# migoox/genome-downsampler

Measured on AMD Instinct MI355X. Metric: Mreads/s selected at target coverage M=100, higher is better.
Workload: dtype u32

## Files before the change

### genome-downsampler_amd/__init__.py

```python
import contextlib
import ctypes as C
import fractions
import heapq
import math
import numbers
import operator
import os

import numpy as np

_HERE = os.path.dirname(os.path.abspath(__file__))
LIB_DIR = os.path.join(_HERE, "lib")
HIP_LIB_PATH = os.environ.get("QMCP_HIP_LIB") or os.path.join(LIB_DIR, "libqmcp_hip.so")
HOST_LIB_PATH = os.environ.get("QMCP_HOST_LIB") or os.path.join(LIB_DIR, "libqmcp_host.so")

ABI_SYMBOLS = (
    "qmcp_hip_abi_version", "qmcp_hip_last_error", "qmcp_hip_device_count", "qmcp_hip_create",
    "qmcp_hip_destroy", "qmcp_hip_solve_host", "qmcp_hip_solve_device", "qmcp_hip_coverage_host",
    "qmcp_hip_filtered_coverage_host", "qmcp_hip_complete_pairs_device",
    "qmcp_hip_complete_pairs_host", "qmcp_hip_amplicon_filter_host", "qmcp_hip_set_profiling",
    "qmcp_hip_kernel_times", "qmcp_hip_filter_solve_host", "qmcp_hip_solve_device_begin",
    "qmcp_hip_solve_end", "qmcp_hip_demand_host", "qmcp_hip_solve_host64", "qmcp_hip_multi_create",
    "qmcp_hip_multi_destroy", "qmcp_hip_multi_solve_host", "qmcp_hip_kept_indices_host",
    "qmcp_hip_default_options", "qmcp_hip_set_options", "qmcp_hip_get_options",
# ... 52 lines not shown
NO_TIER = 0xFFFFFFFF
TIERS_MAX = 16
STRATUM_TALLY_TILE = 1024


QMCP_OK, QMCP_EINVAL, QMCP_EREAD, QMCP_ERANGE, QMCP_ENODEVICE, QMCP_EHIP, QMCP_ENOMEM = 0, -1, -2, -3, -4, -5, -6


class QmcpError(RuntimeError):
    def __init__(self, code, message):
        super().__init__(f"qmcp_hip error {code}: {message}")
        self.code = code


class HostBreakdown(C.Structure):
    _fields_ = [("ms_total", C.c_float), ("ms_narrow_h2d", C.c_float), ("ms_solve", C.c_float),
                ("ms_d2h", C.c_float), ("host_threads", C.c_uint32), ("chunks", C.c_uint32),
                ("columns_sent", C.c_uint32)]


class Stats(C.Structure):
    _fields_ = [
        ("n_reads", C.c_uint64), ("n_kept", C.c_uint64), ("total_length", C.c_uint64),
        ("n_contigs", C.c_uint32), ("path", C.c_uint32), ("min_span", C.c_uint32),
        ("max_span", C.c_uint32), ("sort_passes", C.c_uint32), ("sweep_stretches", C.c_uint32),
        ("ms_total", C.c_float), ("ms_prepare", C.c_float), ("ms_scan", C.c_float),
        ("ms_sort", C.c_float), ("ms_sweep", C.c_float), ("ms_mark", C.c_float),
        ("ms_h2d", C.c_float), ("ms_d2h", C.c_float), ("columns_sent", C.c_uint32),
        ("spec_boundaries", C.c_uint32), ("spec_mismatches", C.c_uint32),
        ("spec_retry_mismatches", C.c_uint32), ("sweep_blocks_changed", C.c_uint32), ("sweep_blocks", C.c_uint32),
        ("arena_grown_mid_solve", C.c_uint32), ("near_uniform_exceptions", C.c_uint32),
        ("near_uniform_selected", C.c_uint32), ("near_uniform_rounds", C.c_uint32),
        ("near_uniform_giveup", C.c_uint32), ("pm_grid", C.c_int32), ("pm_heaviest_wave_slots", C.c_uint32),
    ]

    def as_dict(self):
        return {name: getattr(self, name) for name, _ in self._fields_}


class QualityStats(C.Structure):
    _fields_ = [("quality_min", C.c_uint32), ("quality_max", C.c_uint32), ("key_bits", C.c_uint32),
                ("sort_passes", C.c_uint32), ("cells_contested", C.c_uint64), ("reads_swapped", C.c_uint64),
                ("ms_quality", C.c_float)]

    def as_dict(self):
        return {name: getattr(self, name) for name, _ in self._fields_}


class TargetStats(C.Structure):
    _fields_ = [("reads_on_target", C.c_uint64), ("reads_off_target", C.c_uint64), ("target_positions", C.c_uint64),
                ("regions_in", C.c_uint32), ("regions_merged", C.c_uint32), ("ms_targets", C.c_float)]

    def as_dict(self):
        return {name: getattr(self, name) for name, _ in self._fields_}


class ProfileStats(C.Structure):
    _fields_ = [("positions_in_regions", C.c_uint64), ("capped_positions", C.c_uint64), ("demand", C.c_uint64),
                ("regions_in", C.c_uint32), ("regions_used", C.c_uint32), ("ms_profile", C.c_float)]

    def as_dict(self):
        return {name: getattr(self, name) for name, _ in self._fields_}


class CeilingStats(C.Structure):
    _fields_ = [("reads_placed", C.c_uint64), ("reads_dropped", C.c_uint64), ("mates_dropped", C.c_uint64),
# ... 264 lines not shown


class AmpliconsStats(C.Structure):
    _fields_ = [("units", C.c_uint64), ("units_assigned", C.c_uint64), ("units_filtered", C.c_uint64),
                ("units_no_amplicon", C.c_uint64), ("units_in_several", C.c_uint64), ("reads_shortened", C.c_uint64),
                ("reads_clipped_away", C.c_uint64), ("bases_clipped", C.c_uint64), ("amplicons", C.c_uint64),
                ("amplicons_unused", C.c_uint64), ("ms_assign", C.c_float), ("ms_report", C.c_float)]

    def as_dict(self):
        return {name: getattr(self, name) for name, _ in self._fields_}


assert C.sizeof(AmpliconsStats) == 10 * 8 + 2 * 4


class DepthReport:

    def __init__(self, contig_rows, region_rows, hist_in, hist_kept, stats):
        self.contig_rows, self.region_rows = contig_rows, region_rows
        self.hist_in, self.hist_kept, self.stats = hist_in, hist_kept, stats

    @property
    def valid(self):
        return self.stats.deficit_positions == 0


class Options(C.Structure):
    _fields_ = [
        ("struct_size", C.c_uint32), ("pass_major", C.c_int32), ("sweep", C.c_int32), ("cut_points", C.c_int32),
        ("speculation", C.c_int32), ("speculation_run_in", C.c_uint32), ("near_uniform", C.c_int32),
        ("near_uniform_rounds", C.c_uint32), ("near_uniform_min_depth", C.c_float), ("near_uniform_debug", C.c_int32),
        ("force_sort_route", C.c_int32), ("keep_expand", C.c_int32), ("mixed_sweep_in_lds", C.c_int32),
        ("rank_min_reads", C.c_uint32), ("host_threads", C.c_uint32), ("copy_streams", C.c_uint32),
        ("host_both_columns", C.c_int32), ("pm_grid", C.c_int32),
    ]


class DownsampleRequest(C.Structure):
    _fields_ = (
        [("struct_size", C.c_uint64)]
        + [(name, C.c_char_p) for name in ("solver_name", "in_path", "out_path", "filtered_path", "bed", "tsv", "targets",
                                           "report", "track", "track_channel")]
        + [("ladder_levels", C.POINTER(C.c_uint32))]
        + [(name, C.c_char_p) for name in ("ladder_template", "stratify", "strata_report", "dedup_report")]
        + [(name, C.POINTER(C.c_uint32)) for name in ("region_offsets", "region_starts", "region_ends", "region_caps")]
        + [("n_refs", C.c_uint64), ("pair_stages", C.POINTER(C.c_uint32)), ("template_stages", C.POINTER(C.c_uint32)),
           ("fragment_report", C.c_char_p), ("ceiling_report", C.c_char_p), ("budget_report", C.c_char_p),
           ("budget_reads", C.c_uint64), ("budget_fraction", C.c_double), ("mean_depth_targets", C.c_char_p),
           ("mean_depth_report", C.c_char_p), ("budget_bases", C.c_uint64), ("mean_depth", C.c_double),
           ("thresholds_tag", C.c_char_p), ("thresholds_report", C.c_char_p),
           ("replicates_further", C.POINTER(C.c_uint32)),
           ("replicates_template", C.c_char_p), ("replicates_report", C.c_char_p)]
        + [(name, C.c_uint32) for name in ("max_coverage", "min_len", "min_mapq", "target_padding", "report_bins",
                                           "track_cap", "n_ladder_levels", "default_cap", "n_pair_stages",
                                           "n_template_stages", "n_replicates_further", "thresholds_lo",
                                           "thresholds_hi")]
        + [(name, C.c_int32) for name in ("amplicon_mode", "per_reference", "amplicons_by_reference", "keep_off_target",
                                          "dedup", "has_regions", "pair_aware", "template_aware", "split_spliced",
                                          "include_secondary", "fragment_depth", "ceiling", "has_budget_reads",
                                          "has_budget_bases", "has_mean_depth", "has_replicates", "has_thresholds",
                                          "start_cap_by_strand")]
        + [("start_cap", C.c_uint32), ("start_cap_report", C.c_char_p)]
        + [("primer_clip", C.c_int32), ("per_amplicon", C.c_int32), ("amplicon_report", C.c_char_p)]
        + [("mapq_tiers", C.POINTER(C.c_uint32)), ("n_mapq_tiers", C.c_uint32), ("tiers_report", C.c_char_p)]
        + [("proportional_report", C.c_char_p), ("proportion_num", C.c_uint32), ("proportion_den", C.c_uint32),
           ("proportion_floor", C.c_uint32), ("has_proportion", C.c_int32)])

# ... 2333 lines not shown
```

### genome-downsampler_amd/csrc/api/solve_head.inc.hip

```cpp
int queue_rm_head(qmcp_hip_ctx* c, hipStream_t s1, uint32_t filter, bool clear_mask);
int queue_pm_head(qmcp_hip_ctx* c, hipStream_t st, uint32_t filter, bool rerun);

bool pm_route_ok(const qmcp_hip_ctx* c, const uint64_t* roff, const Problem& pr, uint32_t shift, const qmcp::PmGridPlan& grid) {
    if (c->opt.pass_major < 0) return false;
    const uint32_t n = (uint32_t)pr.n;
    if ((uint64_t)qmcp::pm_slots(n, grid.n_ranges) >= (1ull << 31)) return false;
    if (c->opt.pass_major > 0) return true;
    double slots = 0.0;
    for (uint32_t k = 0; k < pr.n_contigs; ++k) {
        const uint64_t reads = roff[k + 1] - roff[k];
        if (reads == 0 || pr.poff[k + 1] == pr.poff[k]) continue;
        const double ranges = grid.aligned ? (double)((pr.poff[k + 1] - pr.poff[k] + ((1ull << shift) - 1)) >> shift)
                                           : (double)(((pr.poff[k + 1] - 1) >> shift) - (pr.poff[k] >> shift) + 1);
        const double passes = (double)reads / (double)qmcp::pm_pass() < 1.0 ? 1.0 : (double)reads / (double)qmcp::pm_pass();
        const double slice = (double)reads / (passes * ranges);
        slots += passes * ranges * std::ceil(slice / 64.0);
    }
    return slots <= 1.3 * ((double)n / 64.0);
}

int size_arena(qmcp_hip_ctx* c, SolveRun& run, qmcp::PmGridPlan& grid) {
    const Problem& pr = run.pr;
    const uint32_t n = (uint32_t)pr.n, ltot = (uint32_t)pr.ltot, n_contigs = run.n_contigs;
    const uint32_t tiles_seg = qmcp::seg_tile_bound(n);
// ... 195 lines not shown
    uint32_t* d_range_start = c->ranges.u32();
    uint32_t* d_max_load = qmcp::words::max_load(d_range_start);
    {
        KernelSpan sp(c, "k_pm_prepare_sort", st);
        qmcp::launch_pm_prepare_sort(st, run.d_starts, run.d_ends, n, c->roff.u64(), c->poff.u64(),
                                     n_contigs, run.range_shift, run.pm_ranges, d_grid, c->keys[0].as<uint16_t>(), c->keys[1].as<uint16_t>(),
                                     c->hist2.u32(), c->hist.u32(), d_stats, (unsigned long long*)run.d_mask, filter,
                                     filter ? c->nu_exc.u32() : nullptr, nu_cap_for(n),
                                     filter ? qmcp::nu_exc_counts(c->nu_exc.u32(), nu_cap_for(n)) : nullptr);
    }
    HIP_TRY(hipGetLastError());
    HIP_TRY(hipEventRecord(c->ev[EV_PREP], st));
    {
        KernelSpan sp(c, "k_pm_row_sums", st);
        qmcp::launch_pm_row_sums(st, c->hist2.u32(), c->hist.u32(), n, c->pm_work.u32());
    }
    {
        KernelSpan sp(c, "k_pm_tables", st);
        qmcp::launch_pm_tables(st, c->hist2.u32(), c->hist.u32(), n, run.pm_ranges,
                               c->pm_desc.u32(), c->pm_work.u32(), d_range_start, d_max_load,
                               rerun ? nullptr : c->scalars.u32());
    }
    HIP_TRY(hipEventRecord(c->ev_fork, st));
    {
        KernelSpan sp(c, "k_pm_offsets", st);
        qmcp::launch_pm_offsets(st, c->keys[0].as<uint16_t>(), c->pm_desc.u32(), c->hist2.u32(), n,
                                d_range_start, run.range_shift, run.pm_ranges, d_grid, ltot, c->boff.u32(), d_empty);
    }
    HIP_TRY(hipGetLastError());
    run.nu_filter = filter;
    return QMCP_OK;
}

void queue_rank(qmcp_hip_ctx* c, hipStream_t st, const uint32_t* ev_sev, const uint32_t* ev_lastns, uint32_t ell) {
    SolveRun& run = c->run;
    const uint32_t n = (uint32_t)run.pr.n, ltot = (uint32_t)run.pr.ltot;
    if (!run.pm) {
        KernelSpan sp(c, "k_rank_mark");
        qmcp::launch_rank_mark(st, c->keys[0].as<uint16_t>(), c->vals[0].u32(), c->ranges.u32(), run.range_shift, ltot,
                               c->boff.u32(), c->selend.u32(), (unsigned long long*)run.d_mask, c->scalars.as<unsigned long long>(),
                               c->rankamb.p, qmcp::rank_scratch_by_records(run.range_shift, ltot, n));
        return;
    }
    const bool by_records = qmcp::pm_rank_scratch_by_records(run.range_shift, run.pm_ranges, n);
    KernelSpan sp(c, "k_pm_walk", st);
    qmcp::launch_pm_walk(st, c->keys[0].as<uint16_t>(), c->keys[1].as<uint16_t>(), c->pm_desc.u32(), c->hist2.u32(), n,
                         c->ranges.u32(), run.range_shift, run.pm_ranges, c->pm_grid.u32(), c->boff.u32(),
                         c->selend.u32(), (unsigned long long*)run.d_mask, c->scalars.as<unsigned long long>(),
                         c->rankamb.p, by_records, ev_sev, ev_lastns, c->poff.u64(), run.n_contigs, ell);
}
```

### genome-downsampler_amd/csrc/api/solve_tail.inc.hip

```cpp

struct HeadFacts {
    uint32_t min_span, max_span;
    uint32_t max_load;
    uint32_t empty_positions;
    bool uniform;
};

int close_solve(qmcp_hip_ctx* c, bool whole_contigs = false) {
    namespace w = qmcp::words;
    SolveRun& run = c->run;
    TRY(queue_result_scalars(c));
    c->pend_spiky = run.ranked_counted;
    if (run.ranked_counted) {
        HIP_TRY(hipMemcpyAsync(c->h_scalars + w::kHostEmptyPositions, c->stats.u32() + w::kEmptyPositions, sizeof(uint32_t),
                               hipMemcpyDeviceToHost, c->stream));
        c->mem.spiky = Shape{run.n64, run.pr.ltot};
    }
    c->pend_stats = run.local;
    c->pend_M = run.M;
    c->pend_whole_contig_chains = whole_contigs ? whole_contig_chains(run.lengths, run.n_contigs) : 0u;
    c->pending = true;
    return QMCP_OK;
}

// ... 275 lines not shown
        c->mem.spec_hopeless = Shape{local.n_reads, local.total_length, c->pend_M};
    }
    phase_times(c, local);
    local.arena_grown_mid_solve = c->grew_mid_solve;
    if (st) *st = local;
    return QMCP_OK;
}

int solve_complete(qmcp_hip_ctx* c, qmcp_hip_stats* st) { return collect_one(c, st); }

void options_from_env(qmcp_hip_options& o) {
    auto num = [](const char* name) -> uint32_t { const char* e = std::getenv(name); return e ? (uint32_t)std::strtoul(e, nullptr, 10) : 0u; };
    auto flag = [](const char* name) -> int32_t { return std::getenv(name) != nullptr ? 1 : 0; };
    auto tri = [](const char* name) -> int32_t { const char* e = std::getenv(name); return !e ? 0 : e[0] == '1' ? 1 : e[0] == '0' ? -1 : 0; };
    o.pass_major = tri("QMCP_HIP_PM");
    if (const char* e = std::getenv("QMCP_HIP_SWEEP"))
        o.sweep = std::strcmp(e, "fast") == 0 ? QMCP_SWEEP_FAST : std::strcmp(e, "gen") == 0 ? QMCP_SWEEP_GENERAL
                  : std::strcmp(e, "ev") == 0 ? QMCP_SWEEP_EVENTS : QMCP_SWEEP_AUTO;
    o.cut_points = tri("QMCP_HIP_CUTS");
    o.speculation = tri("QMCP_HIP_SPEC");
    o.speculation_run_in = num("QMCP_HIP_SPEC_BURN");
    o.near_uniform = tri("QMCP_HIP_NEAR") < 0 ? -1 : 0;
    o.near_uniform_rounds = num("QMCP_HIP_NEAR_ROUNDS");
    if (const char* e = std::getenv("QMCP_HIP_NEAR_MIN_DEPTH")) o.near_uniform_min_depth = (float)std::strtod(e, nullptr);
    o.near_uniform_debug = flag("QMCP_HIP_NEAR_DEBUG");
    o.force_sort_route = flag("QMCP_HIP_NO_RANK");
    o.keep_expand = flag("QMCP_HIP_EXPAND");
    o.mixed_sweep_in_lds = flag("QMCP_HIP_GENERAL_LDS");
    o.rank_min_reads = num("QMCP_HIP_RANK_MIN");
    o.host_threads = num("QMCP_HIP_HOST_THREADS");
    o.copy_streams = num("QMCP_HIP_COPY_STREAMS");
    o.host_both_columns = flag("QMCP_HIP_HOST_BOTH_COLUMNS");
    if (const char* e = std::getenv("QMCP_HIP_PM_GRID")) o.pm_grid = e[0] == '-' ? -1 : e[0] == '1' || e[0] == '+' ? 1 : 0;
}

int create_ctx(int device, qmcp_hip_ctx** out_ctx) {
    if (!out_ctx) return fail(QMCP_EINVAL, "out_ctx is null");
    *out_ctx = nullptr;
    int n = 0;
    if (hipGetDeviceCount(&n) != hipSuccess || n <= 0) {
        (void)hipGetLastError();
        return fail(QMCP_ENODEVICE, "no HIP device available (quasi-mcp-hip has no CPU fallback)");
    }
    if (device < 0 || device >= n) return fail(QMCP_ENODEVICE, "device %d out of range [0,%d)", device, n);
    HIP_TRY(hipSetDevice(device));
    qmcp_hip_ctx* c = new (std::nothrow) qmcp_hip_ctx();
    if (!c) return fail(QMCP_ENOMEM, "host allocation failed");
    c->device = device;
    qmcp_hip_default_options(&c->opt);
    options_from_env(c->opt);
    hipError_t e = hipStreamCreateWithFlags(&c->stream.h, hipStreamNonBlocking);
    for (int i = 0; e == hipSuccess && i < EV_COUNT; ++i) e = hipEventCreate(&c->ev[i].h);
    if (e == hipSuccess) e = hipEventCreateWithFlags(&c->ev_in.h, hipEventDisableTiming);
    if (e == hipSuccess) {
        int lo = 0, hi = 0;
        (void)hipDeviceGetStreamPriorityRange(&lo, &hi);
        e = hipStreamCreateWithPriority(&c->stream2.h, hipStreamNonBlocking, hi);
    }
    if (e == hipSuccess) e = hipEventCreateWithFlags(&c->ev_fork.h, hipEventDisableTiming);
    if (e == hipSuccess) e = hipEventCreateWithFlags(&c->ev_head.h, hipEventDisableTiming);
    if (e == hipSuccess) e = hipEventCreateWithFlags(&c->ev_done.h, hipEventDisableTiming);
    int rc = e == hipSuccess ? ensure_pinned(c, c->h_head, qmcp::words::kHeadWords * sizeof(uint32_t))
                             : fail(QMCP_EHIP, "context setup: %s", hipGetErrorString(e));
    if (rc != QMCP_OK) {
        qmcp_hip_destroy(c);
        return rc;
// ... 40 lines not shown
```

### genome-downsampler_amd/csrc/kernels/pass_major.inc.hip

```cpp
static constexpr int kPmPass = 8192;
__host__ __device__ inline uint32_t pm_stride_of(uint32_t n_ranges) { return (uint32_t)kPmPass + 64u * n_ranges; }
static constexpr int kPmThreads = 512;
static constexpr int kPmWaves = kPmThreads / 64;
static constexpr int kPmPassesPerWg = 4;
static constexpr size_t kPmSortLds = ((size_t)kPmPass + kPmWaves * 256 + 2 * 256 + 16 + 2 * kPmPassesPerWg * 256 + kPmWaves * 3 * 128) * sizeof(uint32_t);
static constexpr uint32_t kPmExcPerWave = 128;

static constexpr uint32_t kPmFlatDigits = 32;
static constexpr uint32_t kPmStageWords = 10240;
static constexpr uint32_t kPmFlatSlots = 8;
static_assert(kPmStageWords >= (uint32_t)kPmPass + kPmFlatDigits * 63u, "a padded pass of 32 slices fits the stage");
static_assert(kPmStageWords <= (uint32_t)kPmPass + kPmWaves * 3u * kPmExcPerWave, "the stage's tail aliases s_exc and nothing else");
static_assert(kPmFlatDigits == 1u << kPmLaneFormBits, "a pass the lane counts rank is a pass the flat write-out takes");

#ifndef QMCP_PM_MIN_WAVES
#define QMCP_PM_MIN_WAVES 4
#endif
__global__ __launch_bounds__(kPmThreads, QMCP_PM_MIN_WAVES) void k_pm_prepare_sort(
    const uint32_t* __restrict__ starts, const uint32_t* __restrict__ ends, uint32_t n,
    const uint64_t* __restrict__ contig_read_off, const uint64_t* __restrict__ contig_pos_off, uint32_t n_contigs,
    const uint32_t* __restrict__ vbase ,
    uint32_t shift, uint32_t stride ,
    uint16_t* __restrict__ keys16, uint16_t* __restrict__ idx16,
    uint32_t* __restrict__ cnt_tab, uint32_t* __restrict__ lst_tab, uint32_t pitch ,
// ... 876 lines not shown
#pragma unroll
        for (int k = 0; k < kRankDepth - 1; ++k) S[k] = slot_of(d0[k], (uint32_t)k);
        S[kRankDepth - 1] = Slot{0u, 0u, 0u, false};
#define QMCP_PM_ASK_KEYS(K) asm volatile("global_load_ushort " QMCP_PM_KEYREG(K) ", %0, %1\n\tglobal_load_ushort " QMCP_PM_IDXREG(K) ", %0, %2" : : "v"((S[K].slot0 + lane) * 2u), "s"(keys16), "s"(idx16) : QMCP_PM_RING, "memory");
#define QMCP_PM_ASK_DSC(K) asm volatile("global_load_dword " QMCP_PM_DSCREG(K) ", %0, %1" : : "v"(desc_offset(7u + (uint32_t)(K))), "s"(desc) : QMCP_PM_RING, "memory");
        QMCP_PM_ASK_KEYS(0) QMCP_PM_ASK_KEYS(1) QMCP_PM_ASK_KEYS(2) QMCP_PM_ASK_KEYS(3) QMCP_PM_ASK_KEYS(4) QMCP_PM_ASK_KEYS(5) QMCP_PM_ASK_KEYS(6)
        QMCP_PM_ASK_DSC(0) QMCP_PM_ASK_DSC(1) QMCP_PM_ASK_DSC(2) QMCP_PM_ASK_DSC(3) QMCP_PM_ASK_DSC(4) QMCP_PM_ASK_DSC(5) QMCP_PM_ASK_DSC(6) QMCP_PM_ASK_DSC(7)
        asm volatile("s_waitcnt vmcnt(0)" : : : QMCP_PM_RING, "memory");
#undef QMCP_PM_ASK_KEYS
#undef QMCP_PM_ASK_DSC
    }
    QMCP_PM_STAMP_AT(1)
    for (uint32_t c0 = 0; c0 < n_chunks; c0 += kRankDepth) {
        QMCP_PM_STEP(0, 7) QMCP_PM_STEP(1, 0) QMCP_PM_STEP(2, 1) QMCP_PM_STEP(3, 2)
        QMCP_PM_STEP(4, 3) QMCP_PM_STEP(5, 4) QMCP_PM_STEP(6, 5) QMCP_PM_STEP(7, 6)
    }
#undef QMCP_PM_STEP
    asm volatile("s_waitcnt vmcnt(0)" : : : QMCP_PM_RING, "memory");
    QMCP_PM_STAMP_AT(2)
    if (lane < cur - flushed) {
        const uint32_t v = ring[(flushed + lane) & 127u];
        atomicOr(&mask[v >> 6], 1ull << (v & 63u));
    }
    kept = cur;
    __syncthreads();
    kept += pm_settle_groups(keys16, idx16, desc, g0, n_ws, stride, amb, s_namb, w, lane, mask);
    if (lane == 0 && kept) atomicAdd(&s_kept, kept);
    __syncthreads();
    QMCP_PM_STAMP_AT(3)
    QMCP_PM_STAMPS_OUT(1)
    if (tid == 0 && s_kept) atomicAdd(kept_total, (unsigned long long)s_kept);
}

#ifdef QMCP_PM_STAMP
extern "C" int qmcp_lab_pm_stamps(unsigned long long* out) {
    return (int)hipMemcpyFromSymbol(out, HIP_SYMBOL(g_pm_stamps), sizeof(g_pm_stamps));
}
#endif
uint32_t pm_pitch(uint32_t n) { return part_pass_pitch(n); }
uint32_t pm_pass() { return (uint32_t)kPmPass; }
uint32_t pm_stride(uint32_t n_ranges) { return pm_stride_of(n_ranges); }
size_t pm_slots(uint32_t n, uint32_t n_ranges) { return (size_t)pm_pitch(n) * pm_stride(n_ranges); }
uint32_t pm_work_words() { return kPmWorkWords; }
uint32_t pm_exc_slots(uint32_t n) { return pm_pitch(n) * kPmWaves * kPmExcPerWave + kNuOverflow; }
bool pm_rank_scratch_by_records(uint32_t shift, uint32_t n_ranges, uint32_t n) { return (size_t)n < ((size_t)n_ranges << shift); }
size_t pm_rank_scratch_bytes(uint32_t shift, uint32_t n_ranges, uint32_t n) {
    const size_t by_pos = (size_t)n_ranges << shift;
    return (by_pos < (size_t)n ? by_pos : (size_t)n) * sizeof(uint2) + 64;
}
void launch_pm_prepare_sort(hipStream_t st, const uint32_t* starts, const uint32_t* ends, uint32_t n,
                            const uint64_t* d_roff, const uint64_t* d_poff, uint32_t n_contigs, uint32_t shift,
                            uint32_t n_ranges, const uint32_t* d_grid,
                            uint16_t* keys16, uint16_t* idx16, uint32_t* cnt_tab, uint32_t* lst_tab,
                            uint32_t* stats, unsigned long long* zero_mask, uint32_t ell_reg, uint32_t* exc,
                            uint32_t exc_cap, uint32_t* exc_cnt) {
    const uint32_t pitch = pm_pitch(n);
    if (pitch == 0) return;
    (void)hipFuncSetAttribute((const void*)k_pm_prepare_sort, hipFuncAttributeMaxDynamicSharedMemorySize, (int)kPmSortLds);
    hipLaunchKernelGGL(k_pm_prepare_sort, dim3(pitch / kPmPassesPerWg), dim3(kPmThreads), kPmSortLds, st, starts, ends, n,
                       d_roff, d_poff, n_contigs, d_grid + 3u * kPmGridRows, shift, pm_stride(n_ranges), keys16, idx16,
                       cnt_tab, lst_tab, pitch, stats, zero_mask, exc != nullptr ? ell_reg : 0u, exc, exc_cap, exc_cnt);
    if (exc != nullptr && ell_reg != 0u)
        hipLaunchKernelGGL(k_nu_count_groups, dim3(32), dim3(256), 0, st, exc_cnt, pitch * kPmWaves, stats);
}
void launch_pm_row_sums(hipStream_t st, const uint32_t* cnt_tab, const uint32_t* lstw, uint32_t n, uint32_t* work) {
    const uint32_t pitch = pm_pitch(n);
    if (pitch == 0) return;
    hipLaunchKernelGGL(k_pm_row_sums, dim3(256, kPmDescrY), dim3(256), 0, st, cnt_tab, lstw, pitch, work);
}
void launch_pm_tables(hipStream_t st, uint32_t* tab, const uint32_t* lstw, uint32_t n, uint32_t n_ranges,
                      uint32_t* desc, const uint32_t* work, uint32_t* range_start, uint32_t* max_load, uint32_t* clear16) {
    const uint32_t pitch = pm_pitch(n);
    if (pitch == 0) return;
    const uint32_t s64 = pm_stride(n_ranges) / 64u;
    hipLaunchKernelGGL(k_pm_tables, dim3(256, kPmDescrY), dim3(256), 0, st, tab, lstw, pitch, pitch * s64, desc, work,
                       range_start, max_load, clear16);
}
void launch_pm_offsets(hipStream_t st, const uint16_t* keys16, const uint32_t* desc, const uint32_t* Tp, uint32_t n,
                       const uint32_t* range_start, uint32_t shift, uint32_t n_ranges, const uint32_t* d_grid, uint32_t ltot,
                       uint32_t* boff, uint32_t* empty_positions) {
    const size_t width = (size_t)1 << shift;
    const size_t lds = (width + width / 32 + 1) * sizeof(uint32_t);
    (void)hipFuncSetAttribute((const void*)k_pm_offsets, hipFuncAttributeMaxDynamicSharedMemorySize, (int)lds);
    hipLaunchKernelGGL(k_pm_offsets, dim3(n_ranges), dim3(1024), lds, st, keys16, desc, Tp, pm_pitch(n), range_start, d_grid,
                       shift, pm_stride(n_ranges), ltot, boff, empty_positions);
}
void launch_pm_walk(hipStream_t st, const uint16_t* keys16, const uint16_t* idx16, const uint32_t* desc, const uint32_t* Tp,
                    uint32_t n, const uint32_t* range_start, uint32_t shift, uint32_t n_ranges, const uint32_t* d_grid,
                    const uint32_t* boff, const uint32_t* selend, unsigned long long* mask, unsigned long long* kept_total, void* scratch,
                    bool scratch_by_records, const uint32_t* ev_sev, const uint32_t* ev_lastns,
                    const uint64_t* d_poff, uint32_t n_contigs, uint32_t ell) {
    const EvQuota evq{ev_sev, ev_lastns, d_poff, n_contigs, ell, pm_div_make(ell)};
    const size_t lds = (((size_t)1 << shift) + 1) * sizeof(uint32_t);
    (void)hipFuncSetAttribute((const void*)k_pm_walk, hipFuncAttributeMaxDynamicSharedMemorySize, (int)lds);
    hipLaunchKernelGGL(k_pm_walk, dim3(n_ranges), dim3(1024), lds, st, keys16, idx16, desc, Tp, pm_pitch(n), range_start, d_grid, shift,
                       pm_stride(n_ranges), boff, selend, evq, mask, (uint2*)scratch, scratch_by_records ? 1 : 0,
                       kept_total);
}
```

### genome-downsampler_amd/csrc/qmcp_kernels.h

```cpp
#ifndef QMCP_KERNELS_H
#define QMCP_KERNELS_H
#include <hip/hip_runtime.h>
#include <stdint.h>

#include "qmcp_hip.h"
#include "sweep_plan.h"
#include "dedup_plan.h"
#include "thresholds_plan.h"
#include "pm_grid_plan.h"

namespace qmcp {

static constexpr uint32_t kMaxLdsRingSpan = 16383;
static constexpr uint32_t kMaxGeneralSpan = (1u << 24) - 1;
static constexpr uint32_t kMaxUniformSpan = 512;
static constexpr uint32_t kMaxCachedSpan = 4032;

void launch_prepare(hipStream_t st, const uint32_t* starts, const uint32_t* ends, uint32_t n,
                    const uint64_t* d_roff, const uint64_t* d_poff, uint32_t n_contigs,
                    const uint64_t* keep_mask, uint32_t* gstart, uint32_t* cstart,
                    uint32_t* stats, uint32_t part_shift,
                    uint32_t* part_hist ,
                    uint32_t* digit0_hist ,
                    uint32_t* global_digit_hist ,
// ... 134 lines not shown
                          uint32_t* empty_positions );
size_t rank_scratch_bytes(uint32_t shift, uint32_t ltot, uint32_t n);
bool rank_scratch_by_records(uint32_t shift, uint32_t ltot, uint32_t n);
void launch_rank_mark(hipStream_t st, const uint16_t* keys16, const uint32_t* idx,
                      const uint32_t* range_start, uint32_t shift, uint32_t ltot, const uint32_t* boff,
                      const uint32_t* selend, unsigned long long* mask, unsigned long long* kept_total,
                      void* scratch, bool scratch_by_records);

uint32_t pm_pitch(uint32_t n);
uint32_t pm_pass();
uint32_t pm_stride(uint32_t n_ranges);
size_t pm_slots(uint32_t n, uint32_t n_ranges);
size_t pm_rank_scratch_bytes(uint32_t shift, uint32_t n_ranges, uint32_t n);
bool pm_rank_scratch_by_records(uint32_t shift, uint32_t n_ranges, uint32_t n);
uint32_t pm_work_words();
void launch_pm_prepare_sort(hipStream_t st, const uint32_t* starts, const uint32_t* ends, uint32_t n,
                            const uint64_t* d_roff, const uint64_t* d_poff, uint32_t n_contigs, uint32_t shift,
                            uint32_t n_ranges, const uint32_t* d_grid, uint16_t* keys16, uint16_t* idx16, uint32_t* cnt_tab, uint32_t* lst_tab,
                            uint32_t* stats, unsigned long long* zero_mask, uint32_t ell_reg = 0, uint32_t* exc = nullptr,
                            uint32_t exc_cap = 0, uint32_t* exc_cnt = nullptr);
uint32_t pm_exc_slots(uint32_t n);
void launch_pm_row_sums(hipStream_t st, const uint32_t* cnt_tab, const uint32_t* lstw, uint32_t n, uint32_t* work);
void launch_pm_tables(hipStream_t st, uint32_t* tab, const uint32_t* lstw, uint32_t n, uint32_t n_ranges,
                      uint32_t* desc, const uint32_t* work, uint32_t* range_start, uint32_t* max_load, uint32_t* clear16);
void launch_pm_offsets(hipStream_t st, const uint16_t* keys16, const uint32_t* desc, const uint32_t* Tp, uint32_t n,
                       const uint32_t* range_start, uint32_t shift, uint32_t n_ranges, const uint32_t* d_grid, uint32_t ltot,
                       uint32_t* boff, uint32_t* empty_positions);
void launch_pm_walk(hipStream_t st, const uint16_t* keys16, const uint16_t* idx16, const uint32_t* desc, const uint32_t* Tp,
                    uint32_t n, const uint32_t* range_start, uint32_t shift, uint32_t n_ranges, const uint32_t* d_grid,
                    const uint32_t* boff, const uint32_t* selend, unsigned long long* mask, unsigned long long* kept_total, void* scratch,
                    bool scratch_by_records,
                    const uint32_t* ev_sev = nullptr, const uint32_t* ev_lastns = nullptr,
                    const uint64_t* d_poff = nullptr, uint32_t n_contigs = 0, uint32_t ell = 0);


void launch_span_mode_share(hipStream_t st, const uint32_t* starts, const uint32_t* ends, uint32_t n, uint32_t* out );
size_t nu_exc_bytes(uint32_t cap);
uint32_t nu_overflow_slots();
uint32_t* nu_exc_counts(uint32_t* exc, uint32_t cap);
void launch_nu_count_span(hipStream_t st, const uint32_t* starts, const uint32_t* ends, uint32_t n, uint32_t span, uint32_t* out);
void launch_nu_setup(hipStream_t st, uint32_t* exc, uint32_t cap, uint32_t n_exc, const uint32_t* n_over ,
                     const uint32_t* boff, uint32_t ltot, uint32_t ell, uint32_t M, uint32_t* ce ,
                     uint32_t* spine, int32_t* nadj , uint32_t* state );
void launch_nu_round(hipStream_t st, uint32_t* exc, uint32_t cap, uint32_t n_exc, const uint32_t* n_over, bool first_round,
                     const uint32_t* boff, const uint32_t* selend, int32_t* nadj, const uint32_t* ce ,
                     const uint64_t* d_poff, uint32_t n_contigs,
                     uint32_t ell, uint32_t M, uint2* suspects, uint32_t suspects_cap, uint32_t* state,
                     unsigned long long* viol_key, uint32_t* viol_idx,
                     const uint32_t* swept_from ,
                     uint32_t* sweep_from_next ,
                     uint32_t ltot, uint32_t* spine ,
                     const uint32_t* seg_exact , uint32_t n_cand,
                     uint32_t* marks_next ,
                     uint32_t* selend_prev ,
                     uint32_t* dirty ,
                     uint32_t* dirty_next,
                     const uint32_t* seg_fine = nullptr ,
                     uint32_t* fine_next = nullptr );
size_t nu_cells_bytes();
size_t nu_suspect_bytes(uint32_t suspects_cap);
void launch_nu_mark_selected(hipStream_t st, uint32_t* exc, uint32_t cap, uint32_t n_exc, const uint32_t* n_over,
                             unsigned long long* mask, unsigned long long* kept_total);

void launch_bc_keys(hipStream_t st, const uint32_t* starts, const uint32_t* ends, const uint32_t* ids, uint32_t n,
                    const uint32_t* lengths, uint32_t n_contigs, uint32_t* keys, uint32_t* err);
void launch_bc_bounds(hipStream_t st, const void* sorted, uint32_t n, uint32_t n_groups, uint32_t* offs);
// ... 270 lines not shown
```

### include/qmcp_hip.h

```cpp
#ifndef QMCP_HIP_H
#define QMCP_HIP_H

#include <stddef.h>
#include <stdint.h>

#ifdef __cplusplus
extern "C" {
#endif

#define QMCP_HIP_ABI_VERSION 5

enum {
    QMCP_OK = 0,
    QMCP_EINVAL = -1,
    QMCP_EREAD = -2,
    QMCP_ERANGE = -3,
    QMCP_ENODEVICE = -4,
    QMCP_EHIP = -5,
    QMCP_ENOMEM = -6
};

enum {
    QMCP_PATH_NONE = 0,
    QMCP_PATH_UNIFORM = 1,
// ... 4 lines not shown
typedef struct qmcp_hip_ctx qmcp_hip_ctx;

typedef struct qmcp_hip_stats {
    uint64_t n_reads;
    uint64_t n_kept;
    uint64_t total_length;
    uint32_t n_contigs;
    uint32_t path;
    uint32_t min_span;
    uint32_t max_span;
    uint32_t sort_passes;
    uint32_t sweep_stretches;
    float ms_total;
    float ms_prepare;
    float ms_scan;
    float ms_sort;
    float ms_sweep;
    float ms_mark;
    float ms_h2d;
    float ms_d2h;
    uint32_t columns_sent;
    uint32_t spec_boundaries;
    uint32_t spec_mismatches;
    uint32_t spec_retry_mismatches;
    uint32_t sweep_blocks_changed;
    uint32_t sweep_blocks;
    uint32_t arena_grown_mid_solve;
    uint32_t near_uniform_exceptions;
    uint32_t near_uniform_selected;
    uint32_t near_uniform_rounds;
    uint32_t near_uniform_giveup;
    int32_t pm_grid;
    uint32_t pm_heaviest_wave_slots;
} qmcp_hip_stats;

enum {
    QMCP_NU_GIVEUP_NONE = 0,
    QMCP_NU_GIVEUP_NOT_TRIED = 1,
    QMCP_NU_GIVEUP_LONGER_READS = 2,
    QMCP_NU_GIVEUP_TOO_MANY = 3,
    QMCP_NU_GIVEUP_HEAVY_RANGE = 4,
    QMCP_NU_GIVEUP_UNMODELLED = 5,
    QMCP_NU_GIVEUP_BUDGET = 6,
    QMCP_NU_GIVEUP_REMEMBERED = 7
};

int qmcp_hip_abi_version(void);
const char* qmcp_hip_last_error(void);

int qmcp_hip_device_count(void);

int qmcp_hip_create(int device, qmcp_hip_ctx** out_ctx);
void qmcp_hip_destroy(qmcp_hip_ctx* ctx);

typedef struct qmcp_hip_options {
    uint32_t struct_size;
    int32_t pass_major;
    int32_t sweep;
    int32_t cut_points;
    int32_t speculation;
    uint32_t speculation_run_in;
    int32_t near_uniform;
    uint32_t near_uniform_rounds;
    float near_uniform_min_depth;
    int32_t near_uniform_debug;
    int32_t force_sort_route;
    int32_t keep_expand;
    int32_t mixed_sweep_in_lds;
    uint32_t rank_min_reads;
    uint32_t host_threads;
    uint32_t copy_streams;
    int32_t host_both_columns;
    int32_t pm_grid;
} qmcp_hip_options;
enum { QMCP_SWEEP_AUTO = 0, QMCP_SWEEP_FAST = 1, QMCP_SWEEP_GENERAL = 2, QMCP_SWEEP_EVENTS = 3 };
void qmcp_hip_default_options(qmcp_hip_options* out);
int qmcp_hip_set_options(qmcp_hip_ctx* ctx, const qmcp_hip_options* options);
int qmcp_hip_get_options(qmcp_hip_ctx* ctx, qmcp_hip_options* out);

int qmcp_hip_set_profiling(qmcp_hip_ctx* ctx, int enabled);
int qmcp_hip_kernel_times(qmcp_hip_ctx* ctx, char* buf, size_t cap);

int qmcp_hip_solve_host(qmcp_hip_ctx* ctx,
                        const uint32_t* starts, const uint32_t* ends, uint64_t n_reads,
                        const uint64_t* contig_read_offsets, const uint32_t* contig_lengths,
                        uint32_t n_contigs, uint32_t max_coverage,
                        uint64_t* keep_mask_out, qmcp_hip_stats* stats);

typedef struct qmcp_hip_host_breakdown {
    float ms_total;
    float ms_narrow_h2d;
    float ms_solve;
    float ms_d2h;
    uint32_t host_threads;
    uint32_t chunks;
    uint32_t columns_sent;
} qmcp_hip_host_breakdown;
int qmcp_hip_solve_host64(qmcp_hip_ctx* ctx,
                          const uint64_t* start_inds, const uint64_t* end_inds, uint64_t n_reads,
                          const uint64_t* contig_read_offsets, const uint32_t* contig_lengths,
                          uint32_t n_contigs, uint32_t max_coverage,
                          uint64_t* keep_mask_out, qmcp_hip_stats* stats,
                          qmcp_hip_host_breakdown* breakdown);

int qmcp_hip_kept_indices_host(qmcp_hip_ctx* ctx, uint64_t n_reads, uint64_t* indices_out, uint64_t capacity,
                               uint64_t* n_out);
// ... 696 lines not shown
```

Before: 137,500.

## Add sift-form pass-major ranking kernel that filters records by live quota

Adds a new k_pm_sift kernel as an alternative to k_pm_walk for the pass-major ranking step. Each round compacts only the records whose start position still has positive quota into LDS, then processes them in chunks with LDS atomic decrements. Only positions whose quota runs out inside a chunk get group-wise tie resolution, and kept reads are buffered in LDS before being OR-ed into the mask. It is chosen automatically when M*ltot is small relative to span*n (phi<=0.25), the low-coverage case where most records can be skipped. The cost is extra block-wide syncs and LDS pressure per round.

```diff
diff --git a/genome-downsampler_amd/__init__.py b/genome-downsampler_amd/__init__.py
--- a/genome-downsampler_amd/__init__.py
+++ b/genome-downsampler_amd/__init__.py
@@ -108,6 +108,7 @@
         ("arena_grown_mid_solve", C.c_uint32), ("near_uniform_exceptions", C.c_uint32),
         ("near_uniform_selected", C.c_uint32), ("near_uniform_rounds", C.c_uint32),
         ("near_uniform_giveup", C.c_uint32), ("pm_grid", C.c_int32), ("pm_heaviest_wave_slots", C.c_uint32),
+        ("pm_walk_form", C.c_uint32),
     ]
 
     def as_dict(self):
@@ -438,7 +439,7 @@
         ("near_uniform_rounds", C.c_uint32), ("near_uniform_min_depth", C.c_float), ("near_uniform_debug", C.c_int32),
         ("force_sort_route", C.c_int32), ("keep_expand", C.c_int32), ("mixed_sweep_in_lds", C.c_int32),
         ("rank_min_reads", C.c_uint32), ("host_threads", C.c_uint32), ("copy_streams", C.c_uint32),
-        ("host_both_columns", C.c_int32), ("pm_grid", C.c_int32),
+        ("host_both_columns", C.c_int32), ("pm_grid", C.c_int32), ("pm_walk", C.c_int32),
     ]
 
 
diff --git a/genome-downsampler_amd/csrc/api/solve_head.inc.hip b/genome-downsampler_amd/csrc/api/solve_head.inc.hip
--- a/genome-downsampler_amd/csrc/api/solve_head.inc.hip
+++ b/genome-downsampler_amd/csrc/api/solve_head.inc.hip
@@ -251,6 +251,14 @@
     return QMCP_OK;
 }
 
+constexpr double kPmSiftPhi = 0.25;
+bool pm_sift_wanted(const qmcp_hip_ctx* c, uint32_t span) {
+    if (c->opt.pm_walk != 0) return c->opt.pm_walk > 0;
+    const SolveRun& run = c->run;
+    if (span == 0 || run.M == 0 || run.pr.n == 0) return false;
+    return (double)run.M * (double)run.pr.ltot <= kPmSiftPhi * (double)span * (double)run.pr.n;
+}
+
 void queue_rank(qmcp_hip_ctx* c, hipStream_t st, const uint32_t* ev_sev, const uint32_t* ev_lastns, uint32_t ell) {
     SolveRun& run = c->run;
     const uint32_t n = (uint32_t)run.pr.n, ltot = (uint32_t)run.pr.ltot;
@@ -263,6 +271,15 @@
     }
     const bool by_records = qmcp::pm_rank_scratch_by_records(run.range_shift, run.pm_ranges, n);
     KernelSpan sp(c, "k_pm_walk", st);
+    if (pm_sift_wanted(c, ell ? ell : run.nu_filter)) {
+        run.local.pm_walk_form = 2;
+        qmcp::launch_pm_sift(st, c->keys[0].as<uint16_t>(), c->keys[1].as<uint16_t>(), c->pm_desc.u32(), c->hist2.u32(), n,
+                             run.range_shift, run.pm_ranges, c->pm_grid.u32(), c->boff.u32(), c->selend.u32(),
+                             (unsigned long long*)run.d_mask, c->scalars.as<unsigned long long>(), ev_sev, ev_lastns,
+                             c->poff.u64(), run.n_contigs, ell);
+        return;
+    }
+    run.local.pm_walk_form = 1;
     qmcp::launch_pm_walk(st, c->keys[0].as<uint16_t>(), c->keys[1].as<uint16_t>(), c->pm_desc.u32(), c->hist2.u32(), n,
                          c->ranges.u32(), run.range_shift, run.pm_ranges, c->pm_grid.u32(), c->boff.u32(),
                          c->selend.u32(), (unsigned long long*)run.d_mask, c->scalars.as<unsigned long long>(),
diff --git a/genome-downsampler_amd/csrc/api/solve_tail.inc.hip b/genome-downsampler_amd/csrc/api/solve_tail.inc.hip
--- a/genome-downsampler_amd/csrc/api/solve_tail.inc.hip
+++ b/genome-downsampler_amd/csrc/api/solve_tail.inc.hip
@@ -331,6 +331,7 @@
     o.copy_streams = num("QMCP_HIP_COPY_STREAMS");
     o.host_both_columns = flag("QMCP_HIP_HOST_BOTH_COLUMNS");
     if (const char* e = std::getenv("QMCP_HIP_PM_GRID")) o.pm_grid = e[0] == '-' ? -1 : e[0] == '1' || e[0] == '+' ? 1 : 0;
+    if (const char* e = std::getenv("QMCP_HIP_PM_WALK")) o.pm_walk = e[0] == '-' ? -1 : e[0] == '1' || e[0] == '+' ? 1 : 0;
 }
 
 int create_ctx(int device, qmcp_hip_ctx** out_ctx) {
diff --git a/genome-downsampler_amd/csrc/kernels/pass_major.inc.hip b/genome-downsampler_amd/csrc/kernels/pass_major.inc.hip
--- a/genome-downsampler_amd/csrc/kernels/pass_major.inc.hip
+++ b/genome-downsampler_amd/csrc/kernels/pass_major.inc.hip
@@ -932,6 +932,186 @@
     if (tid == 0 && s_kept) atomicAdd(kept_total, (unsigned long long)s_kept);
 }
 
+static constexpr uint32_t kPmSiftRound = 64;
+static constexpr uint32_t kPmSiftSlots = 64u * kPmSiftRound;
+static constexpr uint32_t kPmSiftChunk = 1024;
+static constexpr uint32_t kPmSiftPerWave = kPmSiftRound / 16u;
+static constexpr uint32_t kPmSiftDepth = 4;
+static constexpr uint32_t kPmSiftOut = 896;
+static constexpr uint32_t kPmSiftFlush = 512;
+static_assert(kPmSiftPerWave == 4, "a lane takes four slots of one wave-slot: 8 bytes a stream");
+struct PmSiftLds {
+    uint32_t read[kPmSiftSlots];
+    uint16_t key[kPmSiftSlots];
+    uint32_t grp[kPmSiftChunk];
+    uint32_t wtot[2][16];
+    uint32_t ngrp[2], kept;
+    uint32_t out[kPmSiftOut];
+    uint32_t nout;
+};
+static_assert(sizeof(PmSiftLds) + ((size_t(1) << 15) + 1) * sizeof(int32_t) <= 160u * 1024u, "quotas at shift 15 and the round's lists fit a CU's LDS");
+
+__global__ __launch_bounds__(1024) void k_pm_sift(const uint16_t* __restrict__ keys16, const uint16_t* __restrict__ idx16,
+                                                  const uint32_t* __restrict__ desc,
+                                                  const uint32_t* __restrict__ Tp, uint32_t pitch,
+                                                  const uint32_t* __restrict__ grid, uint32_t stride,
+                                                  const uint32_t* __restrict__ boff, const uint32_t* __restrict__ selend,
+                                                  EvQuota evq,
+                                                  unsigned long long* __restrict__ mask,
+                                                  unsigned long long* __restrict__ kept_total) {
+    extern __shared__ int32_t s_q[];
+    __shared__ PmSiftLds s;
+    const uint32_t range = blockIdx.x;
+    const uint32_t pos0 = pm_grid_pos0(grid, range), live = pm_grid_live(grid, range);
+    const uint32_t tid = threadIdx.x, nthreads = blockDim.x;
+    const uint32_t lane = tid & 63u;
+    const uint32_t w = (uint32_t)__builtin_amdgcn_readfirstlane((int)(tid >> 6));
+    const uint32_t lo_p = Tp[(size_t)range * pitch];
+    const uint32_t hi_p = Tp[(size_t)(range + 1) * pitch];
+    if (lo_p >= hi_p) return;
+    const uint32_t g0 = lo_p >> 6, n_ws = (hi_p - lo_p) >> 6;
+    const uint32_t n_rounds = (n_ws + kPmSiftRound - 1u) / kPmSiftRound;
+    const uint32_t sub = lane >> 4, l_in = lane & 15u;
+    struct Rec { uint2 key, idx; uint32_t nv, read0; };
+    auto ws_of = [&](uint32_t r) -> uint32_t { return r * kPmSiftRound + kPmSiftPerWave * w + sub; };
+    auto ask_descriptors = [&](uint32_t r0) -> uint32_t { return desc[g0 + min(ws_of(r0 + l_in), n_ws - 1u)]; };
+    uint32_t dsc16 = ask_descriptors(0u), dsc16_next = ask_descriptors(16u);
+    auto ask_records = [&](uint32_t r) -> Rec {
+        if ((r & 15u) == 0u && r != 0u) {
+            dsc16 = dsc16_next;
+            dsc16_next = ask_descriptors(r + 16u);
+        }
+        const uint32_t dsc = (uint32_t)__shfl((int)dsc16, (int)((lane & 48u) | (r & 15u)), kWave);
+        const PmSlot at = pm_unpack<true>(dsc, ws_of(r) < n_ws, stride);
+        Rec x;
+        x.nv = at.nv;
+        x.read0 = at.pass * (uint32_t)kPmPass;
+        x.key = *reinterpret_cast<const uint2*>(keys16 + at.slot0 + 4u * l_in);
+        x.idx = *reinterpret_cast<const uint2*>(idx16 + at.slot0 + 4u * l_in);
+        return x;
+    };
+    Rec ring[kPmSiftDepth];
+#pragma unroll
+    for (uint32_t k = 0; k + 1u < kPmSiftDepth; ++k) ring[k] = ask_records(k);
+    if (evq.sev != nullptr) {
+        const uint32_t c_range = pm_grid_contig(grid, range);
+        if (c_range != kPmNoContig) pm_event_quotas<16, true>(evq, c_range, pos0, live, tid, nthreads, s_q);
+        else pm_event_quotas<8, false>(evq, c_range, pos0, live, tid, nthreads, s_q);
+    } else
+    for (uint32_t i0 = tid; i0 < live; i0 += 8 * nthreads) {
+        uint32_t a[8], b[8];
+#pragma unroll
+        for (int u = 0; u < 8; ++u) {
+            const uint32_t i = min(i0 + u * nthreads, live - 1);
+            a[u] = selend[pos0 + i];
+            b[u] = boff[pos0 + i];
+        }
+#pragma unroll
+        for (int u = 0; u < 8; ++u)
+            if (i0 + u * nthreads < live) s_q[i0 + u * nthreads] = (int32_t)(a[u] - b[u]);
+    }
+    if (tid == 0) { s.ngrp[0] = 0; s.ngrp[1] = 0; s.kept = 0; s.nout = 0; }
+    __syncthreads();
+
+    const uint64_t gt_mask = lane == 63 ? 0ull : ~((2ull << lane) - 1ull);
+    uint32_t kept = 0;
+    uint32_t cpar = 0;
+    auto mark = [&](uint32_t v) { atomicOr(&mask[v >> 6], 1ull << (v & 63u)); };
+    auto keep_if = [&](bool k, uint32_t v) {
+        const uint64_t m = __ballot(k);
+        if (m == 0) return;
+        const int first = __ffsll((long long)m) - 1;
+        uint32_t base = 0;
+        if ((int)lane == first) base = atomicAdd(&s.nout, (uint32_t)__popcll(m));
+        base = (uint32_t)__builtin_amdgcn_readlane((int)base, first);
+        if (k) {
+            const uint32_t at = base + __builtin_amdgcn_mbcnt_hi((uint32_t)(m >> 32), __builtin_amdgcn_mbcnt_lo((uint32_t)m, 0u));
+            if (at < kPmSiftOut) s.out[at] = v; else mark(v);
+            ++kept;
+        }
+    };
+    auto round = [&](uint32_t r, const Rec& cur, Rec& far) {
+        far = ask_records(r + kPmSiftDepth - 1u);
+        const uint32_t k[4] = {cur.key.x & 0xFFFFu, cur.key.x >> 16, cur.key.y & 0xFFFFu, cur.key.y >> 16};
+        const uint32_t rd[4] = {cur.read0 + (cur.idx.x & 0xFFFFu), cur.read0 + (cur.idx.x >> 16),
+                                cur.read0 + (cur.idx.y & 0xFFFFu), cur.read0 + (cur.idx.y >> 16)};
+        bool live_x[4];
+        uint32_t cnt = 0;
+#pragma unroll
+        for (uint32_t x = 0; x < 4; ++x) {
+            const bool valid = 4u * l_in + x < cur.nv;
+            live_x[x] = valid && s_q[valid ? k[x] : 0u] > 0;
+            cnt += live_x[x] ? 1u : 0u;
+        }
+        const uint32_t incl = wave_incl_scan_add(cnt);
+        const uint32_t par = r & 1u;
+        if (lane == 63) s.wtot[par][w] = incl;
+        __syncthreads();
+        const uint32_t tot_incl = wave_incl_scan_add(lane < 16u ? s.wtot[par][lane] : 0u);
+        const uint32_t total = (uint32_t)__builtin_amdgcn_readlane((int)tot_incl, 15);
+        const uint32_t wbase = tot_incl - (lane < 16u ? s.wtot[par][lane] : 0u);
+        uint32_t at = (uint32_t)__builtin_amdgcn_readlane((int)wbase, (int)w) + incl - cnt;
+        if (total == 0u) return;
+        const uint32_t nout = s.nout;
+        const bool flush = nout >= kPmSiftFlush;
+        if (flush)
+            for (uint32_t i = tid; i < min(nout, kPmSiftOut); i += 1024u) mark(s.out[i]);
+#pragma unroll
+        for (uint32_t x = 0; x < 4; ++x)
+            if (live_x[x]) {
+                s.key[at] = (uint16_t)k[x];
+                s.read[at] = rd[x];
+                ++at;
+            }
+        __syncthreads();
+        for (uint32_t c0 = 0; c0 < total; c0 += kPmSiftChunk, cpar ^= 1u) {
+            const uint32_t cn = min(kPmSiftChunk, total - c0);
+            const bool valid = tid < cn;
+            const uint32_t key = valid ? s.key[c0 + tid] : 0u;
+            int32_t old = 0;
+            if (valid) old = atomicSub(&s_q[key], 1);
+            __syncthreads();
+            int32_t aft = 0;
+            if (valid) aft = s_q[key];
+            if (valid && old == 1 && aft < 0) s.grp[atomicAdd(&s.ngrp[cpar], 1u)] = (key << 16) | (uint32_t)(-aft);
+            if (tid == 0) s.ngrp[cpar ^ 1u] = 0;
+            if (flush && c0 == 0u && tid == 0) s.nout = 0;
+            __syncthreads();
+            keep_if(valid && old > 0 && aft >= 0, valid ? s.read[c0 + tid] : 0u);
+            const uint32_t ngrp = s.ngrp[cpar];
+            if (ngrp != 0u) {
+                const uint32_t steps = (cn + 63u) >> 6;
+                for (uint32_t g = w; g < ngrp; g += 16u) {
+                    const uint32_t ent = s.grp[g], p = ent >> 16;
+                    uint32_t skip = ent & 0xFFFFu;
+                    for (uint32_t t = steps; t-- != 0u;) {
+                        const uint32_t i = 64u * t + lane;
+                        const bool member = i < cn && s.key[c0 + i] == p;
+                        const uint64_t m = __ballot(member);
+                        if (m == 0) continue;
+                        const uint32_t above = (uint32_t)__popcll(m & gt_mask);
+                        keep_if(member && above >= skip, member ? s.read[c0 + i] : 0u);
+                        const uint32_t in_step = (uint32_t)__popcll(m);
+                        skip = skip > in_step ? skip - in_step : 0u;
+                    }
+                }
+            }
+        }
+    };
+    for (uint32_t r0 = 0; r0 < n_rounds; r0 += kPmSiftDepth) {
+#pragma unroll
+        for (uint32_t k = 0; k < kPmSiftDepth; ++k) {
+            if (r0 + k >= n_rounds) break;
+            round(r0 + k, ring[k], ring[(k + kPmSiftDepth - 1u) % kPmSiftDepth]);
+        }
+    }
+    kept = wave_sum_u32(kept);
+    if (lane == 0 && kept) atomicAdd(&s.kept, kept);
+    __syncthreads();
+    for (uint32_t i = tid; i < min(s.nout, kPmSiftOut); i += 1024u) mark(s.out[i]);
+    if (tid == 0 && s.kept) atomicAdd(kept_total, (unsigned long long)s.kept);
+}
+
 #ifdef QMCP_PM_STAMP
 extern "C" int qmcp_lab_pm_stamps(unsigned long long* out) {
     return (int)hipMemcpyFromSymbol(out, HIP_SYMBOL(g_pm_stamps), sizeof(g_pm_stamps));
@@ -997,3 +1177,13 @@
                        pm_stride(n_ranges), boff, selend, evq, mask, (uint2*)scratch, scratch_by_records ? 1 : 0,
                        kept_total);
 }
+void launch_pm_sift(hipStream_t st, const uint16_t* keys16, const uint16_t* idx16, const uint32_t* desc, const uint32_t* Tp,
+                    uint32_t n, uint32_t shift, uint32_t n_ranges, const uint32_t* d_grid,
+                    const uint32_t* boff, const uint32_t* selend, unsigned long long* mask, unsigned long long* kept_total,
+                    const uint32_t* ev_sev, const uint32_t* ev_lastns, const uint64_t* d_poff, uint32_t n_contigs, uint32_t ell) {
+    const EvQuota evq{ev_sev, ev_lastns, d_poff, n_contigs, ell, pm_div_make(ell)};
+    const size_t lds = (((size_t)1 << shift) + 1) * sizeof(uint32_t);
+    (void)hipFuncSetAttribute((const void*)k_pm_sift, hipFuncAttributeMaxDynamicSharedMemorySize, (int)lds);
+    hipLaunchKernelGGL(k_pm_sift, dim3(n_ranges), dim3(1024), lds, st, keys16, idx16, desc, Tp, pm_pitch(n), d_grid,
+                       pm_stride(n_ranges), boff, selend, evq, mask, kept_total);
+}
diff --git a/genome-downsampler_amd/csrc/qmcp_kernels.h b/genome-downsampler_amd/csrc/qmcp_kernels.h
--- a/genome-downsampler_amd/csrc/qmcp_kernels.h
+++ b/genome-downsampler_amd/csrc/qmcp_kernels.h
@@ -190,6 +190,11 @@
                     bool scratch_by_records,
                     const uint32_t* ev_sev = nullptr, const uint32_t* ev_lastns = nullptr,
                     const uint64_t* d_poff = nullptr, uint32_t n_contigs = 0, uint32_t ell = 0);
+void launch_pm_sift(hipStream_t st, const uint16_t* keys16, const uint16_t* idx16, const uint32_t* desc, const uint32_t* Tp,
+                    uint32_t n, uint32_t shift, uint32_t n_ranges, const uint32_t* d_grid,
+                    const uint32_t* boff, const uint32_t* selend, unsigned long long* mask, unsigned long long* kept_total,
+                    const uint32_t* ev_sev = nullptr, const uint32_t* ev_lastns = nullptr,
+                    const uint64_t* d_poff = nullptr, uint32_t n_contigs = 0, uint32_t ell = 0);
 
 
 void launch_span_mode_share(hipStream_t st, const uint32_t* starts, const uint32_t* ends, uint32_t n, uint32_t* out );
diff --git a/include/qmcp_hip.h b/include/qmcp_hip.h
--- a/include/qmcp_hip.h
+++ b/include/qmcp_hip.h
@@ -60,6 +60,7 @@
     uint32_t near_uniform_giveup;
     int32_t pm_grid;
     uint32_t pm_heaviest_wave_slots;
+    uint32_t pm_walk_form;
 } qmcp_hip_stats;
 
 enum {
@@ -100,6 +101,7 @@
     uint32_t copy_streams;
     int32_t host_both_columns;
     int32_t pm_grid;
+    int32_t pm_walk;
 } qmcp_hip_options;
 enum { QMCP_SWEEP_AUTO = 0, QMCP_SWEEP_FAST = 1, QMCP_SWEEP_GENERAL = 2, QMCP_SWEEP_EVENTS = 3 };
 void qmcp_hip_default_options(qmcp_hip_options* out);
diff --git a/lab/pm_sift_phi.py b/lab/pm_sift_phi.py
--- /dev/null
+++ b/lab/pm_sift_phi.py
@@ -0,0 +1,80 @@
+import argparse
+import hashlib
+import importlib
+import os
+import sys
+
+import numpy as np
+
+R = os.path.dirname(os.path.dirname(os.path.abspath(__file__)))
+sys.path.insert(0, R)
+pkg = importlib.import_module("genome-downsampler_amd")
+import torch
+
+
+def shape_cfg4():
+    ss, ee = [], []
+    for c in range(8):
+        a, b = pkg.reads_gen(0, 6_250_000, 1_000_000, 150, seed=12345 + c)
+        ss.append(a); ee.append(b)
+    return np.concatenate(ss), np.concatenate(ee), np.full(8, 1_000_000, np.uint32), np.arange(9, dtype=np.uint64) * 12_500_000
+
+
+def shape_cfg5_cut():
+    a, b = pkg.reads_gen(0, 2_666_667, 8_000_000, 150, seed=777)
+    return a, b, np.full(1, 8_000_000, np.uint32), np.array([0, a.size], np.uint64)
+
+
+def measure(name, shape, Ms, runs, solves):
+    S, E, lengths, offs = shape
+    dS = torch.from_numpy(S.view(np.int32)).cuda(); dE = torch.from_numpy(E.view(np.int32)).cuda()
+    dM = torch.zeros((S.size + 63) // 64, dtype=torch.int64, device="cuda")
+    span = int(E[0]) - int(S[0]) + 1
+    sv = pkg.Solver(0)
+
+    def solve(M):
+        sv.solve_device(dS.data_ptr(), dE.data_ptr(), S.size, lengths, M, dM.data_ptr(), contig_read_offsets=offs)
+
+    for M in Ms:
+        phi = M * float(lengths.sum()) / (span * S.size)
+        rows = {-1: [], 1: []}
+        digests = set()
+        for form in (-1, 1):
+            sv.set_options(pass_major=1, pm_walk=form)
+            for _ in range(2):
+                solve(M)
+        for _ in range(runs):
+            for form in (-1, 1):
+                sv.set_options(pass_major=1, pm_walk=form)
+                sv.set_profiling(1)
+                for _ in range(solves):
+                    solve(M)
+                kt = sv.kernel_times(); sv.set_profiling(0)
+                st = sv.last_stats
+                assert st.pm_walk_form == (2 if form > 0 else 1), st.as_dict()
+                n, ms = kt["k_pm_walk"]
+                rows[form].append((ms / n, st.ms_total))
+                digests.add(hashlib.sha1(dM.cpu().numpy().tobytes()).hexdigest()[:12])
+        sv.set_options(pass_major=1)
+        solve(M)
+        auto = sv.last_stats.pm_walk_form
+        fmt = lambda rs, k: " / ".join("%.4f" % r[k] for r in rs)
+        print("%s M %4d phi %.3f kept %d digests %s automatic form %d" % (name, M, phi, sv.last_stats.n_kept, sorted(digests), auto))
+        print("    ranking ms   walk %s   sift %s" % (fmt(rows[-1], 0), fmt(rows[1], 0)))
+        print("    ms_total     walk %s   sift %s" % (fmt(rows[-1], 1), fmt(rows[1], 1)), flush=True)
+
+
+def main():
+    ap = argparse.ArgumentParser()
+    ap.add_argument("--runs", type=int, default=3)
+    ap.add_argument("--solves", type=int, default=10)
+    ap.add_argument("--only", default="")
+    args = ap.parse_args()
+    if args.only in ("", "cfg4"):
+        measure("cfg4", shape_cfg4(), (100, 200, 400, 800, 1600), args.runs, args.solves)
+    if args.only in ("", "cfg5"):
+        measure("cfg5_cut", shape_cfg5_cut(), (50,), args.runs, args.solves)
+
+
+if __name__ == "__main__":
+    main()
diff --git a/lab/pm_sift_replay.py b/lab/pm_sift_replay.py
--- /dev/null
+++ b/lab/pm_sift_replay.py
@@ -0,0 +1,75 @@
+import argparse
+import importlib
+import os
+import sys
+
+import numpy as np
+
+ROOT = os.path.dirname(os.path.dirname(os.path.abspath(__file__)))
+sys.path.insert(0, ROOT)
+sys.path.insert(0, os.path.join(ROOT, "oracle"))
+PASS, SHIFT, CHUNK = 8192, 15, 1024
+
+
+def replay_range(keys, pass_of, quota, round_ws):
+    q = quota.astype(np.int64).copy()
+    counts = np.bincount(pass_of)
+    padded = (counts + 63) // 64 * 64
+    base = np.concatenate([[0], np.cumsum(padded)[:-1]])
+    first = np.concatenate([[0], np.cumsum(counts)[:-1]])
+    slot = base[pass_of] + (np.arange(keys.size) - first[pass_of])
+    n_ws = int(padded.sum()) // 64
+    rounds = (n_ws + round_ws - 1) // round_ws
+    round_of = slot // (64 * round_ws)
+    edges = np.searchsorted(round_of, np.arange(rounds + 1))
+    survivors = chunks = groups = largest = kept = 0
+    for r in range(rounds):
+        k = keys[edges[r]:edges[r + 1]]
+        k = k[q[k] > 0]
+        survivors += k.size
+        largest = max(largest, k.size)
+        for c0 in range(0, k.size, CHUNK):
+            chunks += 1
+            pos, cnt = np.unique(k[c0:c0 + CHUNK], return_counts=True)
+            before = q[pos]
+            kept += int(np.minimum(cnt, np.maximum(before, 0)).sum())
+            groups += int(((before > 0) & (before < cnt)).sum())
+            q[pos] = before - cnt
+    return {"records": int(keys.size), "wave_slots": n_ws, "rounds": rounds, "survivors": survivors, "chunks": chunks,
+            "walk_chunks": (n_ws + 15) // 16, "groups": groups, "largest_round": largest, "kept": kept}
+
+
+def main():
+    ap = argparse.ArgumentParser()
+    ap.add_argument("--contig", type=int, default=0)
+    ap.add_argument("--M", type=int, default=100)
+    ap.add_argument("--ranges", default="0,7,15,30")
+    ap.add_argument("--round", type=int, default=64)
+    args = ap.parse_args()
+    pkg = importlib.import_module("genome-downsampler_amd")
+    import oracle_py
+    L, rl = 1_000_000, 150
+    s, e = pkg.reads_gen(pkg.KIND_UNIFORM, 6_250_000, L, rl, seed=12345 + args.contig)
+    mask = oracle_py.solve(s, e, L, args.M)
+    bits = np.unpackbits(np.asarray(mask).view(np.uint8), bitorder="little")[:s.size].astype(bool)
+    S = np.bincount(s[bits].astype(np.int64), minlength=L)
+    starts_with_quota = np.count_nonzero(S)
+    print("contig %d: %d reads, kept %d (%.2f %%), positions with S(p) = 0: %.1f %%, records on positions with S(p) > 0: %.1f %%"
+          % (args.contig, s.size, int(bits.sum()), 100.0 * bits.sum() / s.size, 100.0 * (1 - starts_with_quota / L),
+             100.0 * np.count_nonzero(S[s.astype(np.int64)]) / s.size))
+    width = 1 << SHIFT
+    print("range records wave_slots rounds survivors share%% chunks walk_chunks groups largest_round kept")
+    for d in [int(x) for x in args.ranges.split(",")]:
+        sel = np.nonzero((s >> SHIFT) == d)[0]
+        quota = np.zeros(width, np.int64)
+        live = min(width, L - d * width)
+        quota[:live] = S[d * width:d * width + live]
+        f = replay_range((s[sel] & (width - 1)).astype(np.int64), (sel // PASS).astype(np.int64), quota, args.round)
+        assert f["kept"] == int(bits[sel].sum())
+        print("%5d %7d %10d %6d %9d %5.2f %6d %11d %6d %13d %d" % (d, f["records"], f["wave_slots"], f["rounds"], f["survivors"],
+                                                                   100.0 * f["survivors"] / f["records"], f["chunks"], f["walk_chunks"],
+                                                                   f["groups"], f["largest_round"], f["kept"]))
+
+
+if __name__ == "__main__":
+    main()
```

Measured after the change: 134,400. 2.3% lower.
